# octaviogarcia/RaytracingOneWeekend

Measured on AMD Instinct MI355X. Metric: Msamples/s (W×H×spp/s) + achieved HBM GB/s, 1080p@512spp traced scene, higher is better.
Workload: dtype f32; 1 GPU; C1 S-traced 1920x1080, 10496 spp timed (128 spp/step), depth 50; width=1920, height=1080, max_depth=50, parallelism=tile1, gather=RCCL send/recv (om_gather_frame), rccl_library=/usr/local/lib/python3.10/dist-packages/torch/lib/librccl.so, kernel=auto, pipeline=auto, tail_bounce=default, streams=2

## Files before the change

### raytracingoneweekend_amd/csrc/om_tuning.h

```cpp
#pragma once

#ifndef OM_WF_BLOCK
#define OM_WF_BLOCK 512
#endif
#ifndef OM_WF_WAVES
#define OM_WF_WAVES 8
#endif
#ifndef OM_WF_TAIL_SPB
#define OM_WF_TAIL_SPB 2
#endif
#ifndef OM_WF_TAIL_WGS_PER_CU
#define OM_WF_TAIL_WGS_PER_CU 1
#endif
#ifndef OM_WF_MAX_PATHS_LOG2
#define OM_WF_MAX_PATHS_LOG2 27
#endif
#ifndef OM_WF_BATCH_SPP
#define OM_WF_BATCH_SPP 16
#endif
#ifndef OM_WF_MIN_PATHS_LOG2
#define OM_WF_MIN_PATHS_LOG2 25
#endif
#ifndef OM_WF_HYB_BYTES
#define OM_WF_HYB_BYTES 16384
#endif
#ifndef OM_WF_HYBW_BYTES
#define OM_WF_HYBW_BYTES 0
#endif
#ifndef OM_WF_HYB4_BYTES
#define OM_WF_HYB4_BYTES 0
#endif
#ifndef OM_WF_REFILL
#define OM_WF_REFILL 16
#endif
#ifndef OM_WF_TAIL_SHADE
#define OM_WF_TAIL_SHADE 1
#endif
#ifndef OM_WF_TAIL_UNROLL
#define OM_WF_TAIL_UNROLL 24
#endif
#ifndef OM_WF_TAIL_MARCH_WAVES
#define OM_WF_TAIL_MARCH_WAVES 8
#endif
#ifndef OM_WF_TAIL_REFILL
#define OM_WF_TAIL_REFILL OM_WF_REFILL
#endif
#ifndef OM_WF_TAIL_MARCHED
#define OM_WF_TAIL_MARCHED 1
#endif
#ifndef OM_MARCH_UNROLL
#define OM_MARCH_UNROLL 8
#endif
#ifndef OM_WF_ADAPTIVE_BATCHES
#define OM_WF_ADAPTIVE_BATCHES 3
#endif
#ifndef OM_WF_ADAPTIVE_PATHS_LOG2
#define OM_WF_ADAPTIVE_PATHS_LOG2 22
#endif
#ifndef OM_WF_ADAPTIVE_CAP_LOG2
#define OM_WF_ADAPTIVE_CAP_LOG2 26
#endif
#ifndef OM_WF_ADAPTIVE_TAIL
#define OM_WF_ADAPTIVE_TAIL 8
#endif
#ifndef OM_WF_LANES_PER_CU
#define OM_WF_LANES_PER_CU 4096
#endif
#ifndef OM_WF_LANES_PER_CU_WIDE
#define OM_WF_LANES_PER_CU_WIDE 8192
#endif
#ifndef OM_ACC_GROUP
#define OM_ACC_GROUP 8
#endif
#ifndef OM_B2_NODE_STRIDE
#define OM_B2_NODE_STRIDE 80
#endif
#ifndef OM_BARY_TREE_MIN
#define OM_BARY_TREE_MIN 16
#endif
```

### raytracingoneweekend_amd/csrc/om_wavefront.hip

```cpp
#include "om_wavefront.h"

#include <algorithm>
#include <type_traits>

#include "om_device.h"
#include "om_trace.h"
#include "om_tuning.h"

using namespace omd;

namespace omw {

void QueueSet::release() {
    for (int a = 0; a < 2; ++a) {
        for (int b = 0; b < 3; ++b) { if (q[a][b]) (void)hipFree(q[a][b]); q[a][b] = nullptr; }
        if (qr[a]) (void)hipFree(qr[a]); qr[a] = nullptr;
    }
    if (res) (void)hipFree(res);
    if (res_id) (void)hipFree(res_id);
    if (counts) (void)hipFree(counts);
    if (hit) (void)hipFree(hit);
    res = nullptr; res_id = nullptr; counts = nullptr; hit = nullptr;
}

void Buffers::release() {
    for (auto& s : set) s.release();
    if (n0) (void)hipFree(n0);
    n0 = nullptr; n0_cap = 0;
    for (auto& st : side) { if (st) (void)hipStreamDestroy(st); st = nullptr; }

    for (auto e : ev) (void)hipEventDestroy(e);
    ev.clear();
    cap = 0; counts_n = 0; nsets = 0;
}

namespace {

constexpr uint32_t kNoSample = 0xFFFFFFFFu;
enum { TR_BRUTE = 1, TR_CULLED = 2, TR_BVH = 3, TR_SBVH_LDS = 4, TR_SBVH_GLOBAL = 5, TR_BVH2_LDS = 6, TR_BVH2_GLOBAL = 7,
       TR_BVH4_LDS = 8, TR_BVH4_GLOBAL = 9,
       TR_BVH2_WIDE = 10,
       TR_BARY = 16 };
constexpr int tr_base(int tr) { return tr & (TR_BARY - 1); }
constexpr bool tr_bary(int tr) { return (tr & TR_BARY) != 0; }
#define OM_WAVES_ATTR __attribute__((amdgpu_waves_per_eu(OM_WF_WAVES, OM_WF_WAVES)))
constexpr int kBlk = OM_WF_BLOCK;
constexpr int kStackDepth = 24;
constexpr uint32_t kB2Stride = OM_B2_NODE_STRIDE;
static_assert(kB2Stride % 16u == 0u && kB2Stride >= sizeof(OmBvh2Node), "16-B aligned node slots");
static_assert(kB2LdsBudget / sizeof(OmBvh2Node) * (kB2Stride / 16u) < OM_LEAF, "scaled BVH2 child codes stay below OM_LEAF");
template <int TR>
__host__ __device__ inline uint32_t stack_bytes(const OmSceneDev& S) {
    if (tr_base(TR) == TR_BVH2_WIDE) return kBlk * S.b2w_stack * 4u;
    return kBlk * ((tr_base(TR) == TR_BVH4_LDS || tr_base(TR) == TR_BVH4_GLOBAL) ? S.b4_stack : S.b2_stack) * 2u;
}
__host__ __device__ inline uint32_t b2_stage_bytes(const OmSceneDev& S) {
    return (S.n_b2nodes * kB2Stride + S.n_b2leaves * 4u + 15u) & ~15u;
}
constexpr uint32_t kTailSpb = OM_WF_TAIL_SPB;
constexpr uint32_t kTailWgsPerCu = OM_WF_TAIL_WGS_PER_CU;
constexpr uint32_t kWaves = kBlk / 64;
static_assert(kBlk % 64 == 0 && kTailWgsPerCu >= 1u, "whole waves; a tail grid");
constexpr uint32_t kTailDefault = 16;
constexpr uint32_t kTailMarched = OM_WF_TAIL_MARCHED;
constexpr uint32_t kTailL2 = 10;
constexpr uint32_t kTailBigBatch = 24;
__host__ __device__ inline uint32_t hyb_nodes(const OmSceneDev& S) {
    constexpr uint32_t kCap = OM_WF_HYB_BYTES / (uint32_t)sizeof(OmBvh2NodeH);
    return S.b2_lds_bytes ? 0u : (S.n_b2nodes < kCap ? S.n_b2nodes : kCap);
}
static_assert(sizeof(OmBvh2NodeW) == sizeof(OmBvh2NodeH), "wide and half nodes share a buffer");
__host__ __device__ inline const OmBvh2NodeW* wide_nodes(const OmSceneDev& S) { return (const OmBvh2NodeW*)(S.b2h + S.n_b2nodes); }
__host__ __device__ inline uint32_t hybw_nodes(const OmSceneDev& S) {
    constexpr uint32_t kCap = OM_WF_HYBW_BYTES / (uint32_t)sizeof(OmBvh2NodeW);
    return S.n_b2wnodes < kCap ? S.n_b2wnodes : kCap;
}
__host__ __device__ inline uint32_t hyb4_nodes(const OmSceneDev& S) {
    constexpr uint32_t kCap = OM_WF_HYB4_BYTES / (uint32_t)sizeof(OmBvh4NodeH);
    return S.b4_lds_bytes ? 0u : (S.n_b4nodes < kCap ? S.n_b4nodes : kCap);
}
using MarchedC2Lds = MarchedExactLds<2, 1, 1>;
enum { MV_ARRAYS = 0, MV_EXACT_C2_LDS = 1 };
template <int TR>
__host__ __device__ constexpr bool exact_view_built() { return TR == TR_BRUTE || TR == TR_BVH2_LDS; }
__host__ __device__ inline uint32_t seg_capacity(uint64_t paths, uint32_t nseg) {
    const uint64_t c = (paths + nseg - 1) / nseg;
    return (uint32_t)((c + 63u) / 64u * 64u);
}

extern __shared__ __attribute__((aligned(16))) uint4 wf_lds[];

__device__ __forceinline__ uint32_t wave_sum32(uint32_t v) {
#pragma unroll
    for (int off = 32; off > 0; off >>= 1) v += __shfl_xor(v, off, 64);
    return v;
}
__device__ __forceinline__ void flush_counter(unsigned long long* ctr, int slot, uint32_t v) {
    v = wave_sum32(v);
    if (__lane_id() == 0 && v) atomicAdd(&ctr[slot], (unsigned long long)v);
}

struct Seg {
    uint32_t nseg;
    uint32_t segcap;
};

struct AdPlan { uint32_t c, done; };
struct AdCfg {
    uint32_t sample_count;
    uint32_t batches;
    uint32_t paths;
};
__host__ __device__ inline uint32_t ad_batch(uint32_t c, uint32_t done, uint32_t j, const AdCfg& A) {
    if (c == 0u || done >= A.sample_count || j >= A.batches) return 0u;
    const uint32_t rem = A.sample_count - done, left = A.batches - j;
    const uint32_t even = (rem + left - 1u) / left, want = A.paths / c;
    const uint32_t b = even > want ? even : want;
    return b < rem ? b : rem;
}
struct AdList {
    const uint32_t* list;
    const AdPlan* plan;
    uint32_t* list_next;
    AdPlan* plan_next;
    AdCfg A;
    uint32_t j;
};

struct Queue {
    float4* q0; float4* q1; float4* q2; uint4* qr;
};

struct Gen {
    OmCamDev C;
    const float2* jitter;
    const om_pixel_stats* stats;
    const uint32_t* pixels;
    uint32_t n_pixels, by_pixel, batch;
    const uint32_t* n0;
    uint32_t done;
    AdList ad;
    const uint32_t* tile_off;
    const uint16_t* tile_idx;
    const float* tile_tnear;
};

struct Path {
    F3 o, d, cur;
    float depthf;
    uint32_t first_id, seg, slot;
    Rng g;
};

template <class V>
__device__ __forceinline__ V ld4(const V* q) {
    V v;
    v.x = __builtin_nontemporal_load(&q->x); v.y = __builtin_nontemporal_load(&q->y);
    v.z = __builtin_nontemporal_load(&q->z); v.w = __builtin_nontemporal_load(&q->w);
    return v;
}
__device__ __forceinline__ void load_ray(const Queue& Q, uint64_t i, Path& p) {
    const float4 a = ld4(Q.q0 + i), b = ld4(Q.q1 + i);
    p.o = f3(a.x, a.y, a.z); p.depthf = a.w;
    p.d = f3(b.x, b.y, b.z); p.first_id = __float_as_uint(b.w);
}
__device__ __forceinline__ void load_rest(const Queue& Q, uint64_t i, Path& p) {
    const float4 c = ld4(Q.q2 + i);
    const uint4 r = ld4(Q.qr + i);
    p.cur = f3(c.x, c.y, c.z); p.seg = __float_as_uint(c.w);
    p.g.s = r.x; p.g.k = r.y; p.slot = r.z;
}
template <class V>
__device__ __forceinline__ void st4(V* q, V v) {
    __builtin_nontemporal_store(v.x, &q->x); __builtin_nontemporal_store(v.y, &q->y);
    __builtin_nontemporal_store(v.z, &q->z); __builtin_nontemporal_store(v.w, &q->w);
}
__device__ __forceinline__ void store_path(const Queue& Q, uint64_t i, const Path& p) {
    st4(Q.q0 + i, make_float4(p.o.x, p.o.y, p.o.z, p.depthf));
    st4(Q.q1 + i, make_float4(p.d.x, p.d.y, p.d.z, __uint_as_float(p.first_id)));
    st4(Q.q2 + i, make_float4(p.cur.x, p.cur.y, p.cur.z, __uint_as_float(p.seg)));
    st4(Q.qr + i, make_uint4(p.g.s, p.g.k, p.slot, 0u));
}

struct Tracer {
    const OmBvh2Node* b2n;
    const OmBvh2NodeH* h2l;
    const OmBvh2NodeH* h2g;
    uint32_t nl;
    const OmBvh2NodeW* w2l;
    const OmBvh2NodeW* w2g;
    uint32_t* stk32;
    const OmBvh4Node* b4n;
    const OmBvh4NodeH* h4l;
    const OmBvh4NodeH* h4g;
    const uint32_t* bl;
    const OmAffineTest* recs;
    uint16_t* stk;
};

template <int TRF, uint32_t STACKS = 1>
__device__ __forceinline__ Tracer stage_scene(const OmSceneDev& S) {
    constexpr int TR = tr_base(TRF);
    Tracer t;
    t.stk = (uint16_t*)wf_lds + threadIdx.x;
    t.b2n = S.b2nodes; t.b4n = S.b4nodes; t.bl = S.b2leaves; t.recs = S.srecs;
    t.h2l = S.b2h; t.h2g = S.b2h; t.nl = 0;
    t.h4l = S.b4h; t.h4g = S.b4h;
    t.w2l = wide_nodes(S); t.w2g = wide_nodes(S); t.stk32 = (uint32_t*)wf_lds + threadIdx.x;
    if (TR == TR_BVH4_GLOBAL && hyb4_nodes(S)) {
        t.nl = hyb4_nodes(S);
        uint4* dst = wf_lds + STACKS * stack_bytes<TR>(S) / 16u;
        const uint4* sn = (const uint4*)S.b4h;
        for (uint32_t i = threadIdx.x; i < t.nl * (uint32_t)(sizeof(OmBvh4NodeH) / 16u); i += kBlk) dst[i] = sn[i];
        __syncthreads();
        t.h4l = (const OmBvh4NodeH*)dst;
    }
    if (TR == TR_BVH2_WIDE && hybw_nodes(S)) {
        t.nl = hybw_nodes(S);
        uint4* dst = wf_lds + STACKS * stack_bytes<TR>(S) / 16u;
        const uint4* sn = (const uint4*)wide_nodes(S);
        for (uint32_t i = threadIdx.x; i < t.nl * (uint32_t)(sizeof(OmBvh2NodeW) / 16u); i += kBlk) dst[i] = sn[i];
        __syncthreads();
        t.w2l = (const OmBvh2NodeW*)dst;
    }
    if (TR == TR_BVH2_GLOBAL && hyb_nodes(S)) {
        t.nl = hyb_nodes(S);
        uint4* dst = wf_lds + STACKS * stack_bytes<TR>(S) / 16u;
        const uint4* sn = (const uint4*)S.b2h;
        for (uint32_t i = threadIdx.x; i < t.nl * (uint32_t)(sizeof(OmBvh2NodeH) / 16u); i += kBlk) dst[i] = sn[i];
        __syncthreads();
        t.h2l = (const OmBvh2NodeH*)dst;
    }
    if (TR == TR_BVH2_LDS || TR == TR_BVH4_LDS) {
        constexpr uint32_t wn = TR == TR_BVH2_LDS ? (uint32_t)(sizeof(OmBvh2Node) / 16u) : (uint32_t)(sizeof(OmBvh4Node) / 16u);
        constexpr uint32_t ws = TR == TR_BVH2_LDS ? kB2Stride / 16u : wn;
        const uint32_t nn = (TR == TR_BVH2_LDS ? S.n_b2nodes : S.n_b4nodes) * wn;
        const uint4* sn = TR == TR_BVH2_LDS ? (const uint4*)S.b2nodes : (const uint4*)S.b4nodes;
        uint4* dst = wf_lds + STACKS * stack_bytes<TR>(S) / 16u;
        for (uint32_t i = threadIdx.x; i < nn; i += kBlk) {
            uint4 v = sn[i];
            if (TR == TR_BVH2_LDS && (i % wn) % 2u == 0u && v.w < OM_LEAF) v.w *= ws;
            dst[(i / wn) * ws + i % wn] = v;
        }
        uint32_t* ldst = (uint32_t*)(dst + nn / wn * ws);
        for (uint32_t i = threadIdx.x; i < S.n_b2leaves; i += kBlk) ldst[i] = S.b2leaves[i];
        __syncthreads();
        t.b2n = (const OmBvh2Node*)dst; t.b4n = (const OmBvh4Node*)dst; t.bl = ldst;
    }
    return t;
}

template <int TRF, class Wk>
__device__ __forceinline__ int trace_traced(const OmSceneDev& S, const Tracer& T, F3 o, F3 d, float tmin, float& closest, Wk& w) {
    constexpr int TR = tr_base(TRF);
    static_assert(Wk::BARY == tr_bary(TRF), "the work policy carries the variant's TR_BARY flag");
    if (TR == TR_BVH4_LDS) return traced_bvh4<kBlk>(S, T.b4n, T.bl, T.recs, T.stk, o, d, tmin, closest, w);
    if (TR == TR_BVH4_GLOBAL)
        return traced_bvh4<kBlk, Wk, true>(S, T.h4l, T.bl, T.recs, T.stk, o, d, tmin, closest, w, T.h4g, T.nl);
    if (TR == TR_BVH2_LDS)
        return traced_bvh2<kStackDepth, kBlk, Wk, false, OmBvh2Node, 16>(S, T.b2n, T.bl, T.recs, T.stk, o, d, tmin, closest, w);
    if (TR == TR_BVH2_GLOBAL)
        return traced_bvh2<kStackDepth, kBlk, Wk, true>(S, T.h2l, T.bl, T.recs, T.stk, o, d, tmin, closest, w, T.h2g, T.nl);
    if (TR == TR_BVH2_WIDE)
        return traced_bvh2<(int)kB2WideStack, kBlk, Wk, true>(S, T.w2l, T.bl, T.recs, T.stk32, o, d, tmin, closest, w, T.w2g, T.nl);
    if (TR == TR_SBVH_GLOBAL) return traced_sbvh(S, S.snodes, S.srecs, o, d, tmin, closest, w);
    if (TR == TR_BVH) return traced_bvh(S, o, d, tmin, closest, w);
    return traced_brute<TR == TR_CULLED>(S, o, d, tmin, closest, w);
}

template <int TR, bool MARCH, class Wk>
__device__ __forceinline__ int trace(const OmSceneDev& S, const OmParamsDev& P, const Tracer& T, F3 o, F3 d,
                                     float& closest, Wk& w) {
    closest = P.tmax;
    int best = trace_traced<TR>(S, T, o, d, P.tmin, closest, w);
    if (MARCH) {
        float tm;
        const int mg = march(S, o, d, P.tmin, P.tmax, closest, P.march_steps, tm, w);
        if (mg >= 0) { best = mg; closest = tm; }
    }
    return best;
}

template <bool MARCH, bool USER = MARCH>
__device__ __forceinline__ bool shade_path(const OmSceneDev& S, const OmParamsDev& P, uint32_t depth_cap, Path& p,
                                           float closest, int best, float4* __restrict__ res,
                                           uint32_t* __restrict__ res_id) {
    float seg_depth; uint32_t seg_id;
    if (best >= 0) {
        F3 point, normal;
        finalize<MARCH, USER>(S, best, p.o, p.d, P.tmin, closest, point, normal);
        F3 nd, att;
        scatter(S.mats[best], p.d, normal, p.g, nd, att);
        p.cur = mul(p.cur, att);
        p.o = point; p.d = unit(nd);
        seg_depth = closest; seg_id = (uint32_t)best + 1u;
    } else {
        const float t = 0.5f * (p.d.y + 1.0f);
        p.cur = mul(p.cur, f3((1.0f - t) + 0.5f * t, (1.0f - t) + 0.7f * t, (1.0f - t) + 1.0f * t));
        seg_depth = INFINITY; seg_id = 0u;
    }
    bool finished = false;
    F3 result = p.cur;
    float rdepth = 0.0f; uint32_t rid = 0;
    if (p.seg == 0u) {
        p.depthf = seg_depth; p.first_id = seg_id;
        if (isinf(seg_depth)) { finished = true; rdepth = INFINITY; rid = 0u; }
    } else if (isinf(seg_depth)) {
        finished = true; rdepth = p.depthf; rid = p.first_id;
    }
    if (!finished && p.seg + 1u >= depth_cap) {
        finished = true; result = f3(-0.0f, -0.0f, -0.0f); rdepth = p.depthf; rid = p.first_id;
    }
    if (finished) {
        res[p.slot] = make_float4(result.x, result.y, result.z, rdepth);
        res_id[p.slot] = rid;
        return false;
    }
    p.seg += 1u;
    return true;
}

__device__ __forceinline__ bool gen_path(const OmParamsDev& P, const Gen& R, uint32_t stride, uint64_t i, Path& p,
                                         uint32_t& pixel, uint32_t* __restrict__ res_id) {
    const uint32_t s_local = (uint32_t)i / stride, kk = (uint32_t)i - s_local * stride;
    const uint32_t k = R.ad.list ? R.ad.list[kk] : kk;
    pixel = R.pixels[k];
    uint32_t s;
    bool live;
    if (R.n0) {
        const uint32_t v = R.n0[k];
        s = (v & 0x7FFFFFFFu) + R.done + s_local;
        live = s < P.spp_total && !(v >> 31);
    } else {
        const om_pixel_stats& ps = R.stats[R.by_pixel ? pixel : k];
        s = ps.n + s_local;
        live = s < P.spp_total && !(P.adaptive && (ps.flags & 1u));
    }
    if (!live) {
        res_id[i] = kNoSample;
        return false;
    }
    p.g = path_rng(P.skey, pixel, s);
    const uint32_t line = pixel / P.width;
    gen_camera_ray(R.C, P, R.jitter, (float)(pixel - P.width * line), (float)line, s, p.g, p.o, p.d);
    p.cur = f3(1.0f, 1.0f, 1.0f); p.depthf = 0.0f; p.first_id = 0u; p.seg = 0u; p.slot = (uint32_t)i;
    return true;
}

template <int TR, bool COUNT, bool MARCH, bool FIRST, bool HIT = false, bool USER = MARCH>
__global__ __launch_bounds__(kBlk) OM_WAVES_ATTR void k_bounce(OmSceneDev S, OmParamsDev P, Seg G, Gen R, Queue in,
                                                 const uint32_t* __restrict__ count_in, Queue out,
                                                 uint32_t* __restrict__ count_out, float4* __restrict__ res,
                                                 uint32_t* __restrict__ res_id, unsigned long long* __restrict__ counters,
                                                 const float2* __restrict__ hitbuf, uint32_t* __restrict__ tail_next) {
    const uint64_t seg0 = (uint64_t)blockIdx.x * G.segcap;
    uint32_t n, stride = R.n_pixels;
    uint64_t first0 = seg0;
    if (FIRST) {
        if (tail_next && blockIdx.x == 0 && threadIdx.x == 0) *tail_next = 0u;
        uint64_t paths = (uint64_t)R.n_pixels * R.batch;
        if (R.ad.list) {
            const AdPlan pl = uniform_load(R.ad.plan);
            stride = pl.c;
            paths = (uint64_t)pl.c * ad_batch(pl.c, pl.done, R.ad.j, R.ad.A);
            first0 = (uint64_t)blockIdx.x * seg_capacity(paths, G.nseg);
            n = first0 < paths ? (uint32_t)std::min<uint64_t>(seg_capacity(paths, G.nseg), paths - first0) : 0u;
        } else {
            n = seg0 < paths ? (uint32_t)std::min<uint64_t>(G.segcap, paths - seg0) : 0u;
        }
    } else {
        n = count_in[blockIdx.x];
    }
    if (n == 0) {
        if (threadIdx.x == 0) count_out[blockIdx.x] = 0u;
        return;
    }
    __shared__ uint32_t q_next, q_out;
    if (threadIdx.x == 0) { q_next = kBlk / 64u; q_out = 0u; }
    __syncthreads();
    const Tracer T = HIT ? Tracer{} : stage_scene<TR>(S);
    const uint32_t depth_cap = P.max_depth > 1u ? P.max_depth : 1u;
    WorkT<COUNT, false, tr_bary(TR)> w;
    uint32_t segs = 0;
    const uint32_t lane = __lane_id();
    for (uint32_t chunk = __builtin_amdgcn_readfirstlane(threadIdx.x >> 6); chunk * 64u < n;) {
        const uint32_t jj = chunk * 64u + lane;
        bool keep = false;
        Path p;
        uint32_t p_pixel = 0;
        if (jj < n) {
            const uint64_t i = seg0 + jj;
            bool live = true;
            if (FIRST) {
                live = gen_path(P, R, stride, first0 + jj, p, p_pixel, res_id);
            } else {
                load_ray(in, i, p);
                load_rest(in, i, p);
            }
            if (live) {
                float closest;
                int best;
                if (HIT) {
                    const float2 h = hitbuf[i];
                    closest = h.x; best = __float_as_int(h.y);
                } else if (FIRST && (tr_base(TR) == TR_BVH2_LDS || tr_base(TR) == TR_BVH2_GLOBAL || tr_base(TR) == TR_BVH2_WIDE) && R.tile_off) {
                    const uint32_t line = p_pixel / P.width;
                    const uint32_t tile = (p_pixel - line * P.width) / 8u + (line / 8u) * P.tiles_x;
                    closest = P.tmax;
                    const uint32_t t0 = __builtin_amdgcn_readfirstlane(tile);
                    if (__ballot(tile != t0) == 0)
                        best = traced_tiles<true>(S, R.tile_off, R.tile_idx, t0, p.o, p.d, P.tmin, closest, w, R.tile_tnear);
                    else
                        best = traced_tiles(S, R.tile_off, R.tile_idx, tile, p.o, p.d, P.tmin, closest, w);
                    if (MARCH) {
                        float tm;
                        const int mg = march(S, p.o, p.d, P.tmin, P.tmax, closest, P.march_steps, tm, w);
                        if (mg >= 0) { best = mg; closest = tm; }
                    }
                } else {
                    best = trace<TR, MARCH>(S, P, T, p.o, p.d, closest, w);
                }
                keep = shade_path<MARCH, USER>(S, P, depth_cap, p, closest, best, res, res_id);
                if (COUNT) segs++;
            }
        }
        const uint64_t m = __ballot(keep);
        uint32_t obase = 0u, nc = 0u;
        if (lane == 0) {
            obase = m ? atomicAdd(&q_out, (uint32_t)__popcll(m)) : 0u;
            nc = atomicAdd(&q_next, 1u);
        }
        obase = __builtin_amdgcn_readfirstlane(obase);
        chunk = __builtin_amdgcn_readfirstlane(nc);
        if (keep) store_path(out, seg0 + obase + (uint32_t)__popcll(m & ((1ull << lane) - 1ull)), p);
    }
    __syncthreads();
    if (threadIdx.x == 0) count_out[blockIdx.x] = q_out;
    if (COUNT) {
        flush_counter(counters, OMC_SEGMENTS, segs);
        flush_counter(counters, OMC_PRIM_TESTS, w.prim);
        flush_counter(counters, OMC_PRE_TESTS, w.pre);
        flush_counter(counters, OMC_MARCH, w.march);
    }
}

template <bool COUNT>
__global__ __launch_bounds__(kBlk) OM_WAVES_ATTR void k_raygen(OmParamsDev P, Seg G, Gen R, Queue out,
                                                 uint32_t* __restrict__ count_out, uint32_t* __restrict__ res_id) {
    const uint64_t seg0 = (uint64_t)blockIdx.x * G.segcap;
    uint64_t paths = (uint64_t)R.n_pixels * R.batch, first0 = seg0;
    uint32_t n, stride = R.n_pixels;
    if (R.ad.list) {
        const AdPlan pl = uniform_load(R.ad.plan);
        stride = pl.c;
        paths = (uint64_t)pl.c * ad_batch(pl.c, pl.done, R.ad.j, R.ad.A);
        first0 = (uint64_t)blockIdx.x * seg_capacity(paths, G.nseg);
        n = first0 < paths ? (uint32_t)std::min<uint64_t>(seg_capacity(paths, G.nseg), paths - first0) : 0u;
    } else {
        n = seg0 < paths ? (uint32_t)std::min<uint64_t>(G.segcap, paths - seg0) : 0u;
    }
    __shared__ uint32_t q_out;
    if (threadIdx.x == 0) q_out = 0u;
    __syncthreads();
    const uint32_t lane = __lane_id();
    for (uint32_t base = 0; base < n; base += kBlk) {
        const uint32_t jj = base + threadIdx.x;
        Path p;
        uint32_t pixel;
        const bool keep = jj < n && gen_path(P, R, stride, first0 + jj, p, pixel, res_id);
        const uint64_t m = __ballot(keep);
        uint32_t obase = 0u;
        if (lane == 0 && m) obase = atomicAdd(&q_out, (uint32_t)__popcll(m));
        obase = __builtin_amdgcn_readfirstlane(obase);
        if (keep) store_path(out, seg0 + obase + (uint32_t)__popcll(m & ((1ull << lane) - 1ull)), p);
    }
    __syncthreads();
    if (threadIdx.x == 0) count_out[blockIdx.x] = q_out;
}

template <int TR, bool COUNT, class M, class Wk>
__device__ __forceinline__ void march_lanes(const OmSceneDev& S, const OmParamsDev& P, const Tracer& T, const M& m,
                                            const Queue& in, uint64_t seg0, uint32_t n, uint32_t& next,
                                            float2* __restrict__ hit, Wk& w) {
    const uint32_t lane = __lane_id();
    uint32_t j = threadIdx.x;
    bool act = j < n, marching = false;
    bool dry = !act;
    F3 o = f3(0.0f, 0.0f, 0.0f), d = o;
    float t = 0.0f, closest = 0.0f;
    int best = -1;
    uint32_t iters = 0;
    auto start = [&]() {
        const float4 a = in.q0[seg0 + j], b = in.q1[seg0 + j];
        o = f3(a.x, a.y, a.z); d = f3(b.x, b.y, b.z);
        best = trace<TR, false>(S, P, T, o, d, closest, w);
        marching = march_begin(m, o, d, P.tmin, t);
        iters = P.march_steps;
    };
    if (act) start();
    for (;;) {
#pragma unroll
        for (int u = 0; u < OM_MARCH_UNROLL; ++u) {
            if (act) {
                int gi = -1;
                const int r = marching ? march_step(S, m, o, d, P.tmax, closest, t, iters, gi, w) : 2;
                if (r != 0) {
                    if (r == 1) { best = gi; closest = t; }
                    hit[seg0 + j] = make_float2(closest, __int_as_float(best));
                    act = false;
                }
            }
        }
        const uint64_t want = __ballot(!act && !dry), busy = __ballot(act);
        if (want && (__popcll(want) >= OM_WF_REFILL || busy == 0)) {
            uint32_t base = 0u;
            if (lane == 0) base = atomicAdd(&next, (uint32_t)__popcll(want));
            base = __builtin_amdgcn_readfirstlane(base);
            if (!act && !dry) {
                j = base + (uint32_t)__popcll(want & ((1ull << lane) - 1ull));
                if (j < n) { act = true; start(); } else dry = true;
            }
        }
        if (__ballot(act) == 0) break;
    }
}

template <int TR, bool COUNT, int VIEW>
__global__ __launch_bounds__(kBlk) OM_WAVES_ATTR void k_march(OmSceneDev S, OmParamsDev P, Seg G, Queue in,
                                                const uint32_t* __restrict__ count_in, float2* __restrict__ hit,
                                                unsigned long long* __restrict__ counters) {
    const uint32_t n = count_in[blockIdx.x];
    if (n == 0) return;
    const uint64_t seg0 = (uint64_t)blockIdx.x * G.segcap;
    __shared__ uint32_t next;
    if (threadIdx.x == 0) next = kBlk;
    __syncthreads();
    const Tracer T = stage_scene<TR>(S);
    WorkT<COUNT, false, tr_bary(TR)> w;
    if constexpr (VIEW == MV_EXACT_C2_LDS) {
        __shared__ MarchedC2Lds::Block mblock;
        march_lanes<TR, COUNT>(S, P, T, MarchedC2Lds(S, &mblock), in, seg0, n, next, hit, w);
    } else {
        march_lanes<TR, COUNT>(S, P, T, MarchedArrays(S), in, seg0, n, next, hit, w);
    }
    if (COUNT) {
        flush_counter(counters, OMC_PRIM_TESTS, w.prim);
        flush_counter(counters, OMC_PRE_TESTS, w.pre);
        flush_counter(counters, OMC_MARCH, w.march);
    }
}

struct TailSrc {
    const Queue& in;
    const uint32_t* pre;
    uint32_t s0, ns, segcap;
    __device__ __forceinline__ bool load(uint32_t idx, Path& p) const {
        uint32_t lo = 0, hi = ns;
        while (hi - lo > 1u) {
            const uint32_t mid = (lo + hi) >> 1;
            if (pre[mid] <= idx) lo = mid; else hi = mid;
        }
        const uint64_t i = (uint64_t)(s0 + lo) * segcap + (idx - pre[lo]);
        load_ray(in, i, p);
        load_rest(in, i, p);
        return true;
    }
};
template <int TR, bool COUNT, class M, class Src, class Wk>
__device__ __forceinline__ uint32_t tail_march_lanes(const OmSceneDev& S, const OmParamsDev& P, const Tracer& T, const M& m,
                                                     const Src& src, uint32_t total, uint32_t& next,
                                                     float4* __restrict__ res, uint32_t* __restrict__ res_id, Wk& w) {
    const uint32_t lane = __lane_id();
    const uint32_t depth_cap = P.max_depth > 1u ? P.max_depth : 1u;
    uint32_t idx = threadIdx.x, segs = 0, iters = 0;
    bool have = idx < total, dry = !have, marching = false, act = false;
    __shared__ uint32_t rest[9][kBlk];
    Path p;
    float t = 0.0f, closest = 0.0f;
    int best = -1;
    auto park = [&]() {
        const uint32_t i = threadIdx.x;
        rest[0][i] = __float_as_uint(p.cur.x); rest[1][i] = __float_as_uint(p.cur.y); rest[2][i] = __float_as_uint(p.cur.z);
        rest[3][i] = __float_as_uint(p.depthf); rest[4][i] = p.first_id; rest[5][i] = p.seg; rest[6][i] = p.slot;
        rest[7][i] = p.g.s; rest[8][i] = p.g.k;
    };
    auto unpark = [&]() {
        const uint32_t i = threadIdx.x;
        p.cur = f3(__uint_as_float(rest[0][i]), __uint_as_float(rest[1][i]), __uint_as_float(rest[2][i]));
        p.depthf = __uint_as_float(rest[3][i]); p.first_id = rest[4][i]; p.seg = rest[5][i]; p.slot = rest[6][i];
        p.g.s = rest[7][i]; p.g.k = rest[8][i];
    };
    auto begin = [&]() {
        park();
        best = trace<TR, false>(S, P, T, p.o, p.d, closest, w);
        marching = march_begin(m, p.o, p.d, P.tmin, t);
        iters = P.march_steps;
        act = true;
    };
    if (have) { have = src.load(idx, p); if (have) begin(); }
    for (;;) {
#pragma unroll
        for (int u = 0; u < OM_WF_TAIL_UNROLL; ++u) {
            if (act) {
                int gi = -1;
                const int r = marching ? march_step(S, m, p.o, p.d, P.tmax, closest, t, iters, gi, w) : 2;
                if (r != 0) {
                    if (r == 1) { best = gi; closest = t; }
                    act = false;
                }
            }
        }
        const bool ended = have && !act;
        const uint64_t em = __ballot(ended), am = __ballot(act);
        if (ended && (OM_WF_TAIL_SHADE <= 1 || __popcll(em) >= OM_WF_TAIL_SHADE || am == 0)) {
            if (COUNT) segs++;
            unpark();
            if (shade_path<true, M::USER>(S, P, depth_cap, p, closest, best, res, res_id)) begin();
            else have = false;
        }
        const uint64_t want = __ballot(!have && !dry), busy = __ballot(have);
        if (want && (__popcll(want) >= OM_WF_TAIL_REFILL || busy == 0)) {
            uint32_t base = 0u;
// ... 469 lines not shown
    for (uint32_t bounce = 0; bounce < depth_cap; ++bounce) {
        const Queue in = queue(B, bounce & 1u), out = queue(B, (bounce + 1u) & 1u);
        const uint32_t* cin = B.counts + (size_t)bounce * G.nseg;
        if (bounce > 0 && bounce >= tail_at) return tail(in, cin);
        uint32_t* cout = B.counts + (size_t)(bounce + 1u) * G.nseg;
        const int ti = each ? tm.begin(st) : -1;
        if (bounce == 0)
            hipLaunchKernelGGL((k_bounce<TR, COUNT, MARCH, true>), dim3(G.nseg), dim3(kBlk), lds, st, L.S, L.P, G, R, in,
                               cin, out, cout, B.res, B.res_id, L.counters, (const float2*)nullptr, tail_next);
        else
            hipLaunchKernelGGL((k_bounce<TR, COUNT, MARCH, false>), dim3(G.nseg), dim3(kBlk), lds, st, L.S, L.P, G, R, in,
                               cin, out, cout, B.res, B.res_id, L.counters, (const float2*)nullptr, (uint32_t*)nullptr);
        tm.end(ti, bounce == 0 ? OM_KT_BOUNCE0 : OM_KT_BOUNCE, st);
        ++launches;
    }
    return launches;
    }
}

template <int TR>
uint32_t run_tr(bool count, bool march, QueueSet& B, const Launch& L, hipStream_t st, Seg G, const Gen& R,
                uint32_t depth_cap, uint32_t tail_at, uint32_t lds, uint32_t tail_grid) {
    if (count && march) return run_batch<TR, true, true>(B, L, st, G, R, depth_cap, tail_at, lds, tail_grid);
    if (count) return run_batch<TR, true, false>(B, L, st, G, R, depth_cap, tail_at, lds, tail_grid);
    if (march) return run_batch<TR, false, true>(B, L, st, G, R, depth_cap, tail_at, lds, tail_grid);
    return run_batch<TR, false, false>(B, L, st, G, R, depth_cap, tail_at, lds, tail_grid);
}

hipError_t ensure_events(Buffers& B, size_t n) {
    while (B.ev.size() < n) {
        hipEvent_t e = nullptr;
        const hipError_t r = hipEventCreateWithFlags(&e, hipEventDisableTiming);
        if (r != hipSuccess) return r;
        B.ev.push_back(e);
    }
    return hipSuccess;
}

int pick_trace(int trace_mode, const OmSceneDev& S) {
    int tr = trace_mode == TR_SBVH_LDS ? TR_SBVH_GLOBAL : trace_mode;
    if (tr == TR_BVH2_WIDE) {
        if (S.n_b2wnodes) return TR_BVH2_WIDE | TR_BARY;
        tr = TR_BVH2_LDS;
    }
    if (tr == TR_BVH4_LDS) tr = S.n_b4nodes == 0 ? TR_BVH2_LDS : (S.b4_lds_bytes ? TR_BVH4_LDS : TR_BVH4_GLOBAL);
    if (tr == TR_BVH2_LDS && S.n_b2nodes == 0 && S.n_b2wnodes) return TR_BVH2_WIDE | TR_BARY;
    if (tr == TR_BVH2_LDS)
        tr = S.n_b2nodes == 0 ? (S.n_bvh_nodes <= 1u ? TR_BRUTE : TR_BVH) : (S.b2_lds_bytes ? TR_BVH2_LDS : TR_BVH2_GLOBAL);
    const int bary = S.n_srec_bary ? TR_BARY : 0;
    switch (tr) {
        case TR_BRUTE: case TR_CULLED: case TR_BVH: return tr;
        case TR_SBVH_GLOBAL: case TR_BVH2_LDS: case TR_BVH4_LDS: case TR_BVH4_GLOBAL: return tr | bary;
        default: return TR_BVH2_GLOBAL | bary;
    }
}
uint32_t trace_lds(int trf, const OmSceneDev& S) {
    const int tr = tr_base(trf);
    return tr == TR_BVH2_LDS ? stack_bytes<TR_BVH2_LDS>(S) + b2_stage_bytes(S)
         : tr == TR_BVH2_GLOBAL ? stack_bytes<TR_BVH2_GLOBAL>(S) + hyb_nodes(S) * (uint32_t)sizeof(OmBvh2NodeH)
         : tr == TR_BVH4_LDS ? stack_bytes<TR_BVH4_LDS>(S) + S.b4_lds_bytes
         : tr == TR_BVH4_GLOBAL ? stack_bytes<TR_BVH4_GLOBAL>(S) + hyb4_nodes(S) * (uint32_t)sizeof(OmBvh4NodeH)
         : tr == TR_BVH2_WIDE ? stack_bytes<TR_BVH2_WIDE>(S) + hybw_nodes(S) * (uint32_t)sizeof(OmBvh2NodeW)
         : 0u;
}
template <class F>
void with_tr(int tr, F f) {
    switch (tr) {
        case TR_BRUTE: f(std::integral_constant<int, TR_BRUTE>{}); break;
        case TR_CULLED: f(std::integral_constant<int, TR_CULLED>{}); break;
        case TR_BVH: f(std::integral_constant<int, TR_BVH>{}); break;
        case TR_SBVH_GLOBAL: f(std::integral_constant<int, TR_SBVH_GLOBAL>{}); break;
        case TR_BVH2_LDS: f(std::integral_constant<int, TR_BVH2_LDS>{}); break;
        case TR_BVH4_LDS: f(std::integral_constant<int, TR_BVH4_LDS>{}); break;
        case TR_BVH4_GLOBAL: f(std::integral_constant<int, TR_BVH4_GLOBAL>{}); break;
        case TR_SBVH_GLOBAL | TR_BARY: f(std::integral_constant<int, TR_SBVH_GLOBAL | TR_BARY>{}); break;
        case TR_BVH2_LDS | TR_BARY: f(std::integral_constant<int, TR_BVH2_LDS | TR_BARY>{}); break;
        case TR_BVH2_GLOBAL | TR_BARY: f(std::integral_constant<int, TR_BVH2_GLOBAL | TR_BARY>{}); break;
        case TR_BVH4_LDS | TR_BARY: f(std::integral_constant<int, TR_BVH4_LDS | TR_BARY>{}); break;
        case TR_BVH4_GLOBAL | TR_BARY: f(std::integral_constant<int, TR_BVH4_GLOBAL | TR_BARY>{}); break;
        case TR_BVH2_WIDE | TR_BARY: f(std::integral_constant<int, TR_BVH2_WIDE | TR_BARY>{}); break;
        default: f(std::integral_constant<int, TR_BVH2_GLOBAL>{}); break;
    }
}

template <int TR, bool MARCH, bool USER>
void launch_query(const Query& Q, const OmParamsDev& P, uint32_t grid, uint32_t lds, hipStream_t st) {
    if (Q.windows) {
        if (Q.count)
            hipLaunchKernelGGL((k_query_windows<TR, MARCH, USER, true>), dim3(grid), dim3(kBlk), lds, st, Q.S, P, Q.rays, Q.windows, Q.n, Q.hits, Q.counters);
        else
            hipLaunchKernelGGL((k_query_windows<TR, MARCH, USER, false>), dim3(grid), dim3(kBlk), lds, st, Q.S, P, Q.rays, Q.windows, Q.n, Q.hits, Q.counters);
    } else if (Q.count)
        hipLaunchKernelGGL((k_query<TR, MARCH, USER, true>), dim3(grid), dim3(kBlk), lds, st, Q.S, P, Q.rays, Q.n, Q.hits, Q.counters);
    else
        hipLaunchKernelGGL((k_query<TR, MARCH, USER, false>), dim3(grid), dim3(kBlk), lds, st, Q.S, P, Q.rays, Q.n, Q.hits, Q.counters);
}
template <int TR, bool MARCH>
void launch_occluded(const Query& Q, const OmParamsDev& P, uint32_t grid, uint32_t lds, hipStream_t st) {
    if (Q.count)
        hipLaunchKernelGGL((k_occluded<TR, MARCH, true>), dim3(grid), dim3(kBlk), lds, st, Q.S, P, Q.rays, Q.windows, Q.n, Q.occluded, Q.counters);
    else
        hipLaunchKernelGGL((k_occluded<TR, MARCH, false>), dim3(grid), dim3(kBlk), lds, st, Q.S, P, Q.rays, Q.windows, Q.n, Q.occluded, Q.counters);
}

}

hipError_t render(Buffers& B, const Launch& L, hipStream_t st, std::string& err) {
    const uint32_t n_px = L.n_pixels;
    if (n_px == 0 || L.P.sample_count == 0) return hipSuccess;
    const bool adaptive = L.P.adaptive != 0u;
    const uint32_t want = std::max<uint32_t>(1u, std::min<uint32_t>(L.streams, (uint32_t)kMaxSets));
    const uint64_t kMaxPaths = std::min<uint64_t>(1ull << OM_WF_MAX_PATHS_LOG2,
                                                  std::max<uint64_t>(1ull << OM_WF_MIN_PATHS_LOG2, (uint64_t)OM_WF_BATCH_SPP * n_px));
    uint32_t ns, nb, batch = 0, ad_k = 0, cmax = 0;
    uint64_t max_paths;
    std::vector<uint32_t> done_at(1, 0u);
    AdCfg A{};
    if (adaptive) {
        const uint32_t chunks = (n_px + 63u) / 64u;
        ns = std::min<uint32_t>(want, chunks);
        cmax = std::min<uint32_t>(n_px, (chunks + ns - 1u) / ns * 64u);
        const uint64_t capmax = 1ull << OM_WF_ADAPTIVE_CAP_LOG2;
        uint64_t k = L.ad_batches ? L.ad_batches : OM_WF_ADAPTIVE_BATCHES;
        while (k < L.P.sample_count && (uint64_t)cmax * ((L.P.sample_count + k - 1u) / k) > capmax) ++k;
        ad_k = (uint32_t)std::min<uint64_t>(k, L.P.sample_count);
        A.sample_count = L.P.sample_count; A.batches = ad_k;
        A.paths = 1u << (L.ad_paths_log2 ? L.ad_paths_log2 : OM_WF_ADAPTIVE_PATHS_LOG2);
        max_paths = std::max<uint64_t>(std::min<uint64_t>(A.paths, (uint64_t)cmax * L.P.sample_count),
                                       (uint64_t)cmax * ((L.P.sample_count + ad_k - 1u) / ad_k));
        nb = ad_k * ns;
    } else {
        const bool concurrent = want >= 2u && L.P.sample_count >= 2u;
        batch = (uint32_t)std::max<uint64_t>(1, std::min<uint64_t>(L.P.sample_count, kMaxPaths / n_px));
        if (concurrent) batch = std::min<uint32_t>(batch, (L.P.sample_count + want - 1u) / want);
        while (done_at.back() < L.P.sample_count)
            done_at.push_back(done_at.back() + std::min(batch, L.P.sample_count - done_at.back()));
        nb = (uint32_t)done_at.size() - 1u;
        ns = concurrent ? std::min<uint32_t>(want, nb) : 1u;
        max_paths = (uint64_t)n_px * batch;
    }
    const uint32_t depth_cap = L.P.max_depth > 1u ? L.P.max_depth : 1u;
    int dev = 0;
    (void)hipGetDevice(&dev);
    int cus = 256;
    (void)hipDeviceGetAttribute(&cus, hipDeviceAttributeMultiprocessorCount, dev);
    const int tr = pick_trace(L.trace_mode, L.S);
    const bool march = (L.S.n_msph + L.S.n_mbox + L.S.n_mtor + L.S.n_msdf) != 0u;
    const bool l2_tree = tr_base(tr) == TR_BVH2_GLOBAL || tr_base(tr) == TR_BVH4_GLOBAL || tr_base(tr) == TR_BVH2_WIDE;
    const uint32_t tail_at = L.tail_bounce ? L.tail_bounce
                           : march ? kTailMarched : l2_tree ? kTailL2
                           : adaptive ? OM_WF_ADAPTIVE_TAIL
                           : max_paths > (1ull << 25) ? kTailBigBatch : kTailDefault;
    const uint32_t lanes_per_cu = (march || l2_tree) ? OM_WF_LANES_PER_CU_WIDE : OM_WF_LANES_PER_CU;
    uint32_t nseg = (uint32_t)std::min<uint64_t>((max_paths + kBlk - 1) / kBlk, (uint64_t)cus * (lanes_per_cu / kBlk));
    nseg = (nseg + kTailSpb - 1) / kTailSpb * kTailSpb;
    const uint32_t segcap = seg_capacity(max_paths, nseg);
    hipError_t e = grow(B, (uint64_t)nseg * segcap, (depth_cap + 1u) * nseg + 1u, (int)ns);
    if (e != hipSuccess) { err = "wavefront buffer allocation failed"; return e; }
    const uint32_t lds = trace_lds(tr, L.S);
    const uint32_t tail_grid = (uint32_t)cus * kTailWgsPerCu;
    int lds_max = 0;
    (void)hipDeviceGetAttribute(&lds_max, hipDeviceAttributeMaxSharedMemoryPerBlock, dev);
    if (!march && tail_at < depth_cap && tail_lds(lds, nseg) > (uint32_t)lds_max) {
        err = "the tail's LDS request exceeds the device's limit";
        return hipErrorInvalidValue;
    }
    if (lds > (uint32_t)lds_max) {
        err = "the traversal's LDS request exceeds the device's limit";
        return hipErrorInvalidValue;
    }
    Gen R;
    R.C = L.C; R.jitter = L.jitter; R.stats = L.stats; R.pixels = L.pixels; R.n_pixels = n_px;
    R.by_pixel = L.stats_by_pixel ? 1u : 0u;
    R.tile_off = L.tile_off; R.tile_idx = L.tile_idx; R.tile_tnear = L.tile_tnear;
    R.n0 = nullptr; R.done = 0; R.ad = AdList{};
    hipStream_t streams[kMaxSets] = {st, st, st, st};
    Timer& tm = *L.timer;
    const int call_ti = tm.begin(st);
    const uint32_t plan_stride = ad_k + 1u;
    const uint64_t words = adaptive ? (uint64_t)ns * 2u * cmax + (uint64_t)ns * plan_stride * 2u : (ns > 1 ? n_px : 0u);
    if (words > B.n0_cap) {
        if (B.n0) (void)hipFree(B.n0);
        B.n0 = nullptr; B.n0_cap = 0;
        if ((e = hipMalloc(&B.n0, (size_t)words * sizeof(uint32_t))) != hipSuccess) { err = "n0 allocation failed"; return e; }
        B.n0_cap = words;
    }
    uint32_t* lists = B.n0;
    AdPlan* plans = adaptive ? (AdPlan*)(B.n0 + (uint64_t)ns * 2u * cmax) : nullptr;
    if (adaptive) {
        (void)hipMemsetAsync(plans, 0, (size_t)ns * plan_stride * sizeof(AdPlan), st);
        hipLaunchKernelGGL(k_ad_init, dim3((n_px + kAdInitBlk - 1u) / kAdInitBlk), dim3(kAdInitBlk), 0, st, L.stats, L.pixels, n_px, R.by_pixel,
                           L.P.spp_total, ns, lists, (uint64_t)2u * cmax, plans, plan_stride);
    } else if (ns > 1) {
        hipLaunchKernelGGL(k_snapshot, dim3((n_px + 255u) / 256u), dim3(256), 0, st, L.stats, L.pixels, n_px, R.by_pixel, B.n0);
        R.n0 = B.n0;
    }
    if (ns > 1) {
        if ((e = ensure_events(B, kMaxSets + nb)) != hipSuccess) { err = "event creation failed"; return e; }
        (void)hipEventRecord(B.ev[0], st);
        for (uint32_t k = 1; k < ns; ++k) {
            if (!B.side[k] && (e = hipStreamCreateWithFlags(&B.side[k], hipStreamNonBlocking)) != hipSuccess) {
                err = "side stream creation failed"; return e;
            }
            streams[k] = B.side[k];
            (void)hipStreamWaitEvent(streams[k], B.ev[0], 0);
        }
    }
    uint32_t launches = 0;
    for (uint32_t i = 0; i < nb; ++i) {
        const uint32_t sidx = i % ns;
        hipStream_t si = streams[sidx];
        QueueSet& QS = B.set[sidx];
        Seg G;
        G.nseg = nseg;
        uint32_t b = 0, grid_a;
        AdList ad{};
        if (adaptive) {
            const uint32_t j = i / ns;
            uint32_t* lbase = lists + (uint64_t)sidx * 2u * cmax;
            ad.list = lbase + (uint64_t)(j & 1u) * cmax;
            ad.list_next = lbase + (uint64_t)((j + 1u) & 1u) * cmax;
            ad.plan = plans + (uint64_t)sidx * plan_stride + j;
            ad.plan_next = plans + (uint64_t)sidx * plan_stride + j + 1u;
            ad.A = A; ad.j = j;
            G.segcap = segcap;
            grid_a = (cmax + kBlk - 1) / kBlk;
        } else {
            const uint32_t done = done_at[i];
            b = done_at[i + 1] - done;
            G.segcap = seg_capacity((uint64_t)n_px * b, nseg);
            R.done = done;
            grid_a = (n_px + kBlk - 1) / kBlk;
        }
        R.batch = b;
        R.ad = ad;
        with_tr(tr, [&](auto t) {
            launches += run_tr<decltype(t)::value>(L.count, march, QS, L, si, G, R, depth_cap, tail_at, lds, tail_grid);
        });
        if (ns > 1 && i > 0) (void)hipStreamWaitEvent(si, B.ev[kMaxSets + i - 1u], 0);
        const int ati = tm.mode == 1 ? tm.begin(si) : -1;
        if (L.count)
            hipLaunchKernelGGL(k_accumulate<true>, dim3(grid_a), dim3(kBlk), 0, si, L.P, L.stats, L.pixels, n_px,
                               L.stats_by_pixel ? 1u : 0u, b, QS.res, QS.res_id, L.S.bloom, ad, L.counters);
        else
            hipLaunchKernelGGL(k_accumulate<false>, dim3(grid_a), dim3(kBlk), 0, si, L.P, L.stats, L.pixels, n_px,
                               L.stats_by_pixel ? 1u : 0u, b, QS.res, QS.res_id, L.S.bloom, ad, L.counters);
        tm.end(ati, OM_KT_ACCUMULATE, si);
        if (L.progress_host)
            (void)hipMemcpyAsync(L.progress_host, L.counters + OMC_PROGRESS, sizeof(unsigned long long),
                                 hipMemcpyDeviceToHost, si);
        if (ns > 1) (void)hipEventRecord(B.ev[kMaxSets + i], si);
        if ((e = hipGetLastError()) != hipSuccess) { err = "wavefront launch failed"; return e; }
    }
    for (uint32_t k = 1; k < ns; ++k) {
        (void)hipEventRecord(B.ev[k], streams[k]);
        (void)hipStreamWaitEvent(st, B.ev[k], 0);
    }
    tm.end(call_ti, OM_KT_BOUNCE_SPAN, st, launches);
    return hipSuccess;
}

uint32_t query_max_grid() {
    int dev = 0;
    (void)hipGetDevice(&dev);
    int cus = 256;
    (void)hipDeviceGetAttribute(&cus, hipDeviceAttributeMultiprocessorCount, dev);
    return (uint32_t)cus * (uint32_t)(OM_WF_WAVES * 4 * 64 / kBlk);
}

void tree_regime(int trace_mode, const OmSceneDev& S, int32_t* regime, uint32_t* lds_bytes) {
    const int tr = pick_trace(trace_mode, S);
    const int b = tr_base(tr);
    const bool asked_b2 = trace_mode == TR_BVH2_LDS || trace_mode == TR_BVH4_LDS || trace_mode == TR_BVH2_WIDE;
    *regime = b == TR_BVH2_LDS ? OM_TREE_LDS : b == TR_BVH2_GLOBAL ? OM_TREE_L2 : b == TR_BVH2_WIDE ? OM_TREE_WIDE
            : (b == TR_BVH && asked_b2) ? OM_TREE_FALLBACK_BVH : OM_TREE_NONE;
    *lds_bytes = trace_lds(tr, S);
}

hipError_t query(const Query& Q, hipStream_t st) {
    if (Q.n == 0) return hipSuccess;
    const int tr = pick_trace(Q.trace_mode, Q.S);
    const uint32_t lds = trace_lds(tr, Q.S);
    {
        int dev = 0, lds_max = 0;
        (void)hipGetDevice(&dev);
        (void)hipDeviceGetAttribute(&lds_max, hipDeviceAttributeMaxSharedMemoryPerBlock, dev);
        if (lds > (uint32_t)lds_max) return hipErrorInvalidValue;
    }
    const bool march = (Q.S.n_msph + Q.S.n_mbox + Q.S.n_mtor + Q.S.n_msdf) != 0u;
    const bool user = Q.S.n_msdf != 0u;
    OmParamsDev P{};
    P.tmin = Q.tmin; P.tmax = Q.tmax; P.march_steps = Q.march_steps;
    const uint32_t grid = (uint32_t)std::min<uint64_t>(((uint64_t)Q.n + kBlk - 1u) / kBlk, query_max_grid());
    with_tr(tr, [&](auto t) {
        constexpr int TR = decltype(t)::value;
        if (Q.occluded) {
            if (march) launch_occluded<TR, true>(Q, P, grid, lds, st);
            else launch_occluded<TR, false>(Q, P, grid, lds, st);
        } else if (user) launch_query<TR, true, true>(Q, P, grid, lds, st);
        else if (march) launch_query<TR, true, false>(Q, P, grid, lds, st);
        else launch_query<TR, false, false>(Q, P, grid, lds, st);
    });
    return hipGetLastError();
}

}
```

Before: 7313 Msamples/s.

## Deal primary path blocks round-robin across segments and halve lanes per CU

Path indices are no longer split into contiguous per-segment ranges. They are dealt in groups of eight 64-path blocks round-robin across segments, so each workgroup generates interleaved pixel and sample ranges in the first bounce and in raygen. The intent is to balance the work per segment, since adjacent pixels have correlated path lengths and termination, and to improve coherence. The default lanes per CU also drops from 4096 to 2048, which halves the number of segments on non-marched scenes. Queue capacity now comes from the deal, and fewer segments risks lower occupancy during later bounces.

```diff
diff --git a/raytracingoneweekend_amd/csrc/om_deal.h b/raytracingoneweekend_amd/csrc/om_deal.h
--- /dev/null
+++ b/raytracingoneweekend_amd/csrc/om_deal.h
@@ -0,0 +1,46 @@
+#pragma once
+#include <cstdint>
+
+#if defined(__HIPCC__) || defined(__CUDACC__)
+#define OM_DEAL_HD __host__ __device__
+#else
+#define OM_DEAL_HD
+#endif
+
+struct Deal {
+    uint64_t paths;
+    uint64_t blocks;
+    uint32_t nseg;
+    uint32_t d;
+
+    OM_DEAL_HD uint64_t groups() const { return (blocks + d - 1u) / d; }
+    OM_DEAL_HD uint32_t blocks_of(uint32_t g) const {
+        const uint64_t ng = groups();
+        if (g >= ng) return 0u;
+        const uint64_t mine = (ng - 1u - g) / nseg + 1u;
+        uint64_t b = mine * d;
+        if ((ng - 1u) % nseg == g) b -= ng * d - blocks;
+        return (uint32_t)b;
+    }
+    OM_DEAL_HD uint64_t block(uint32_t g, uint32_t c) const {
+        return ((uint64_t)(c / d) * nseg + g) * d + c % d;
+    }
+    OM_DEAL_HD uint32_t paths_of(uint32_t g) const {
+        uint64_t n = (uint64_t)blocks_of(g) * 64u;
+        if (blocks && ((blocks - 1u) / d) % nseg == g) n -= blocks * 64u - paths;
+        return (uint32_t)n;
+    }
+    OM_DEAL_HD uint32_t capacity() const {
+        return (uint32_t)((groups() + nseg - 1u) / nseg * d * 64u);
+    }
+};
+
+inline uint32_t deal_segments(uint64_t max_paths, uint32_t cus, uint32_t lanes_per_cu, uint32_t blk, uint32_t spb) {
+    const uint64_t want = (max_paths + blk - 1u) / blk, cap = (uint64_t)cus * (lanes_per_cu / blk);
+    const uint32_t nseg = (uint32_t)(want < cap ? want : cap);
+    return (nseg + spb - 1u) / spb * spb;
+}
+
+OM_DEAL_HD inline Deal make_deal(uint64_t paths, uint32_t nseg, uint32_t d) {
+    return Deal{paths, (paths + 63u) / 64u, nseg, d};
+}
diff --git a/raytracingoneweekend_amd/csrc/om_tuning.h b/raytracingoneweekend_amd/csrc/om_tuning.h
--- a/raytracingoneweekend_amd/csrc/om_tuning.h
+++ b/raytracingoneweekend_amd/csrc/om_tuning.h
@@ -64,10 +64,13 @@
 #define OM_WF_ADAPTIVE_TAIL 8
 #endif
 #ifndef OM_WF_LANES_PER_CU
-#define OM_WF_LANES_PER_CU 4096
+#define OM_WF_LANES_PER_CU 2048
 #endif
 #ifndef OM_WF_LANES_PER_CU_WIDE
 #define OM_WF_LANES_PER_CU_WIDE 8192
+#endif
+#ifndef OM_WF_DEAL_BLOCKS
+#define OM_WF_DEAL_BLOCKS 8
 #endif
 #ifndef OM_ACC_GROUP
 #define OM_ACC_GROUP 8
diff --git a/raytracingoneweekend_amd/csrc/om_wavefront.hip b/raytracingoneweekend_amd/csrc/om_wavefront.hip
--- a/raytracingoneweekend_amd/csrc/om_wavefront.hip
+++ b/raytracingoneweekend_amd/csrc/om_wavefront.hip
@@ -6,6 +6,7 @@
 #include "om_device.h"
 #include "om_trace.h"
 #include "om_tuning.h"
+#include "om_deal.h"
 
 using namespace omd;
 
@@ -83,10 +84,7 @@
 enum { MV_ARRAYS = 0, MV_EXACT_C2_LDS = 1 };
 template <int TR>
 __host__ __device__ constexpr bool exact_view_built() { return TR == TR_BRUTE || TR == TR_BVH2_LDS; }
-__host__ __device__ inline uint32_t seg_capacity(uint64_t paths, uint32_t nseg) {
-    const uint64_t c = (paths + nseg - 1) / nseg;
-    return (uint32_t)((c + 63u) / 64u * 64u);
-}
+__host__ __device__ inline Deal batch_deal(uint64_t paths, uint32_t nseg) { return make_deal(paths, nseg, OM_WF_DEAL_BLOCKS); }
 
 extern __shared__ __attribute__((aligned(16))) uint4 wf_lds[];
 
@@ -355,7 +353,7 @@
                                                  const float2* __restrict__ hitbuf, uint32_t* __restrict__ tail_next) {
     const uint64_t seg0 = (uint64_t)blockIdx.x * G.segcap;
     uint32_t n, stride = R.n_pixels;
-    uint64_t first0 = seg0;
+    Deal dl{};
     if (FIRST) {
         if (tail_next && blockIdx.x == 0 && threadIdx.x == 0) *tail_next = 0u;
         uint64_t paths = (uint64_t)R.n_pixels * R.batch;
@@ -363,11 +361,9 @@
             const AdPlan pl = uniform_load(R.ad.plan);
             stride = pl.c;
             paths = (uint64_t)pl.c * ad_batch(pl.c, pl.done, R.ad.j, R.ad.A);
-            first0 = (uint64_t)blockIdx.x * seg_capacity(paths, G.nseg);
-            n = first0 < paths ? (uint32_t)std::min<uint64_t>(seg_capacity(paths, G.nseg), paths - first0) : 0u;
-        } else {
-            n = seg0 < paths ? (uint32_t)std::min<uint64_t>(G.segcap, paths - seg0) : 0u;
-        }
+        }
+        dl = batch_deal(paths, G.nseg);
+        n = dl.blocks_of(blockIdx.x);
     } else {
         n = count_in[blockIdx.x];
     }
@@ -383,16 +379,16 @@
     WorkT<COUNT, false, tr_bary(TR)> w;
     uint32_t segs = 0;
     const uint32_t lane = __lane_id();
-    for (uint32_t chunk = __builtin_amdgcn_readfirstlane(threadIdx.x >> 6); chunk * 64u < n;) {
-        const uint32_t jj = chunk * 64u + lane;
+    const uint32_t chunks = FIRST ? n : (n + 63u) / 64u;
+    for (uint32_t chunk = __builtin_amdgcn_readfirstlane(threadIdx.x >> 6); chunk < chunks;) {
+        const uint64_t i = FIRST ? dl.block(blockIdx.x, chunk) * 64u + lane : seg0 + chunk * 64u + lane;
         bool keep = false;
         Path p;
         uint32_t p_pixel = 0;
-        if (jj < n) {
-            const uint64_t i = seg0 + jj;
+        if (FIRST ? i < dl.paths : chunk * 64u + lane < n) {
             bool live = true;
             if (FIRST) {
-                live = gen_path(P, R, stride, first0 + jj, p, p_pixel, res_id);
+                live = gen_path(P, R, stride, i, p, p_pixel, res_id);
             } else {
                 load_ray(in, i, p);
                 load_rest(in, i, p);
@@ -448,26 +444,24 @@
 __global__ __launch_bounds__(kBlk) OM_WAVES_ATTR void k_raygen(OmParamsDev P, Seg G, Gen R, Queue out,
                                                  uint32_t* __restrict__ count_out, uint32_t* __restrict__ res_id) {
     const uint64_t seg0 = (uint64_t)blockIdx.x * G.segcap;
-    uint64_t paths = (uint64_t)R.n_pixels * R.batch, first0 = seg0;
-    uint32_t n, stride = R.n_pixels;
+    uint64_t paths = (uint64_t)R.n_pixels * R.batch;
+    uint32_t stride = R.n_pixels;
     if (R.ad.list) {
         const AdPlan pl = uniform_load(R.ad.plan);
         stride = pl.c;
         paths = (uint64_t)pl.c * ad_batch(pl.c, pl.done, R.ad.j, R.ad.A);
-        first0 = (uint64_t)blockIdx.x * seg_capacity(paths, G.nseg);
-        n = first0 < paths ? (uint32_t)std::min<uint64_t>(seg_capacity(paths, G.nseg), paths - first0) : 0u;
-    } else {
-        n = seg0 < paths ? (uint32_t)std::min<uint64_t>(G.segcap, paths - seg0) : 0u;
-    }
+    }
+    const Deal dl = batch_deal(paths, G.nseg);
+    const uint32_t nblk = dl.blocks_of(blockIdx.x);
     __shared__ uint32_t q_out;
     if (threadIdx.x == 0) q_out = 0u;
     __syncthreads();
     const uint32_t lane = __lane_id();
-    for (uint32_t base = 0; base < n; base += kBlk) {
-        const uint32_t jj = base + threadIdx.x;
+    for (uint32_t c = threadIdx.x >> 6; c < nblk; c += kBlk / 64u) {
+        const uint64_t i = dl.block(blockIdx.x, c) * 64u + lane;
         Path p;
         uint32_t pixel;
-        const bool keep = jj < n && gen_path(P, R, stride, first0 + jj, p, pixel, res_id);
+        const bool keep = i < dl.paths && gen_path(P, R, stride, i, p, pixel, res_id);
         const uint64_t m = __ballot(keep);
         uint32_t obase = 0u;
         if (lane == 0 && m) obase = atomicAdd(&q_out, (uint32_t)__popcll(m));
@@ -1243,9 +1237,8 @@
                            : adaptive ? OM_WF_ADAPTIVE_TAIL
                            : max_paths > (1ull << 25) ? kTailBigBatch : kTailDefault;
     const uint32_t lanes_per_cu = (march || l2_tree) ? OM_WF_LANES_PER_CU_WIDE : OM_WF_LANES_PER_CU;
-    uint32_t nseg = (uint32_t)std::min<uint64_t>((max_paths + kBlk - 1) / kBlk, (uint64_t)cus * (lanes_per_cu / kBlk));
-    nseg = (nseg + kTailSpb - 1) / kTailSpb * kTailSpb;
-    const uint32_t segcap = seg_capacity(max_paths, nseg);
+    const uint32_t nseg = deal_segments(max_paths, (uint32_t)cus, lanes_per_cu, kBlk, kTailSpb);
+    const uint32_t segcap = batch_deal(max_paths, nseg).capacity();
     hipError_t e = grow(B, (uint64_t)nseg * segcap, (depth_cap + 1u) * nseg + 1u, (int)ns);
     if (e != hipSuccess) { err = "wavefront buffer allocation failed"; return e; }
     const uint32_t lds = trace_lds(tr, L.S);
@@ -1319,7 +1312,7 @@
         } else {
             const uint32_t done = done_at[i];
             b = done_at[i + 1] - done;
-            G.segcap = seg_capacity((uint64_t)n_px * b, nseg);
+            G.segcap = batch_deal((uint64_t)n_px * b, nseg).capacity();
             R.done = done;
             grid_a = (n_px + kBlk - 1) / kBlk;
         }
```

After: 7712 Msamples/s, median of 6. 1.05x the previous value.
